# ray-project/anyscale-workshop-nyc-2023

Measured on NVIDIA H100. Metric: generated tokens/sec (and prompts/sec) FLAN-T5-base 512->128, higher is better.
Workload: dtype bf16

## Files before the change

anyscale_workshop_nyc_2023_b200/csrc/attention_encoder.cuh:

```cuda
#pragma once
#include "attention_decode.cuh"
#include "ptx.cuh"

namespace b200 {

constexpr int kEncThreads = 128;
constexpr int kEncQ = 64;
constexpr int kEncKC = 64;
constexpr int kEncPackMaxS = 512;

DEVINL void cp_async_16(uint32_t smem_dst, const void* gsrc, bool valid) {
  const int sz = valid ? 16 : 0;
  asm volatile("cp.async.cg.shared.global [%0], [%1], 16, %2;" ::"r"(smem_dst), "l"(gsrc), "r"(sz) : "memory");
}
DEVINL void cp_async_commit() { asm volatile("cp.async.commit_group;" ::: "memory"); }
template <int N>
DEVINL void cp_async_wait() {
  asm volatile("cp.async.wait_group %0;" ::"n"(N) : "memory");
}
DEVINL void ldmatrix_x4(uint32_t addr, uint32_t& r0, uint32_t& r1, uint32_t& r2, uint32_t& r3) {
  asm volatile("ldmatrix.sync.aligned.m8n8.x4.shared.b16 {%0,%1,%2,%3}, [%4];"
               : "=r"(r0), "=r"(r1), "=r"(r2), "=r"(r3)
               : "r"(addr));
}
// ... 157 lines not shown
          float cm = -INFINITY;
#pragma unroll
          for (int nt = 0; nt < 8; ++nt) cm = fmaxf(cm, fmaxf(sacc[nt][2 * r], sacc[nt][2 * r + 1]));
          cm = fmaxf(cm, __shfl_xor_sync(0xffffffffu, cm, 1));
          cm = fmaxf(cm, __shfl_xor_sync(0xffffffffu, cm, 2));
          const float mn = fmaxf(m_run[r], cm);
          float add = 0.f;
#pragma unroll
          for (int nt = 0; nt < 8; ++nt) add += expf(sacc[nt][2 * r] - mn) + expf(sacc[nt][2 * r + 1] - mn);
          l_run[r] = l_run[r] * expf(m_run[r] - mn) + add;
          m_run[r] = mn;
        }
      } else {
        const uint32_t vbase = sV_u + buf * 8192;
#pragma unroll
        for (int kk = 0; kk < 4; ++kk) {
          uint32_t pa[4];
          pa[0] = pack_act2(expf(sacc[2 * kk][0] - m_run[0]) / l_run[0], expf(sacc[2 * kk][1] - m_run[0]) / l_run[0]);
          pa[1] = pack_act2(expf(sacc[2 * kk][2] - m_run[1]) / l_run[1], expf(sacc[2 * kk][3] - m_run[1]) / l_run[1]);
          pa[2] = pack_act2(expf(sacc[2 * kk + 1][0] - m_run[0]) / l_run[0],
                              expf(sacc[2 * kk + 1][1] - m_run[0]) / l_run[0]);
          pa[3] = pack_act2(expf(sacc[2 * kk + 1][2] - m_run[1]) / l_run[1],
                              expf(sacc[2 * kk + 1][3] - m_run[1]) / l_run[1]);
#pragma unroll
          for (int dp = 0; dp < 4; ++dp) {
            const int mi = lane >> 3;
            const int key = kk * 16 + (mi & 1) * 8 + (lane & 7);
            const int ch = dp * 2 + (mi >> 1);
            uint32_t b0, b1, b2, b3;
            ldmatrix_x4_trans(vbase + tile_off(key, ch), b0, b1, b2, b3);
            mma_act_16816(oacc[2 * dp], pa, b0, b1);
            mma_act_16816(oacc[2 * dp + 1], pa, b2, b3);
          }
        }
      }
      __syncthreads();
    }
  }

#pragma unroll
  for (int r = 0; r < 2; ++r) {
    const int i = i0 + row_l0 + r * 8;
    if (i < rows) {
      act_t* dst = ctx + (row0 + i) * I + h * 64 + tq * 2;
#pragma unroll
      for (int nt = 0; nt < 8; ++nt)
        *reinterpret_cast<uint32_t*>(dst + nt * 8) = pack_act2(oacc[nt][2 * r], oacc[nt][2 * r + 1]);
    }
  }
}

inline size_t encoder_attn_smem_bytes(int S) { return 8192 + 16384 + 16384 + (S + 64) * 4 + S + 16; }

}
```

anyscale_workshop_nyc_2023_b200/csrc/b200t5.cu:

```cuda
#include <cuda.h>
#include <cuda_bf16.h>
#include <cuda_fp16.h>
#include <cuda_runtime.h>
#include <math.h>
#include <stdarg.h>
#include <stdio.h>
#include <string.h>

#include <algorithm>
#include <map>
#include <memory>
#include <string>
#include <vector>

#include "../../include/b200t5.h"
#include "attention_decode.cuh"
#include "attention_cross_stream.cuh"
#include "attention_encoder.cuh"
#include "elementwise.cuh"
#include "gemm.cuh"
#include "gemm_splitk.cuh"
#include "gemm_2cta.cuh"

using namespace b200;
// ... 283 lines not shown
  long long g_eos = -1, g_pad = -1;
  int g_min_new = -1;
  long long* h_ids = nullptr;
  long long* h_mask = nullptr;
  long long* h_out = nullptr;
  int* h_len = nullptr;
  DecodeState* h_state = nullptr;
  ~Plan() {
    if (gexec) cudaGraphExecDestroy(gexec);
    if (graph) cudaGraphDestroy(graph);
    if (gexec8) cudaGraphExecDestroy(gexec8);
    if (graph8) cudaGraphDestroy(graph8);
    if (h_ids) cudaFreeHost(h_ids);
    if (h_mask) cudaFreeHost(h_mask);
    if (h_out) cudaFreeHost(h_out);
    if (h_len) cudaFreeHost(h_len);
    if (h_state) cudaFreeHost(h_state);
    if (h_cu) cudaFreeHost(h_cu);
    if (h_unf) cudaFreeHost(h_unf);
    if (h_admit) cudaFreeHost(h_admit);
  }
};

struct b200t5_ctx {
  Cfg c;
  int device = 0;
  int num_sms = 132;
  bool finalized = false;
  int ffo_k = 0;
  char err[512] = "";
  std::map<std::string, std::unique_ptr<DevBuf>> raw;
  std::map<std::string, std::unique_ptr<DevBuf>> raw_f32;
  std::map<std::string, std::vector<int64_t>> raw_shape;
  DevBuf shared, lm_head, enc_final_ln, dec_final_ln, enc_relbias, dec_relbias, wcrosskv;
  CUtensorMap tm_lm, tm_crosskv, tm2_crosskv;
  std::vector<float> enc_relbias_h, dec_relbias_h;
  std::vector<EncLayerW> enc;
  std::vector<DecLayerW> dec;
  std::unique_ptr<Plan> plan;
  cudaStream_t cap_stream = nullptr, exec_stream = nullptr, enc_stream = nullptr;
  cudaEvent_t enc_done_ev = nullptr, admitted_ev = nullptr;
  bool admit_overlap = true;
  cudaEvent_t ev[4] = {nullptr, nullptr, nullptr, nullptr};
  bool ev_valid = false;
  int pow_mode = 0;
  bool use_pdl = true;
  GeluLut gelu_lut{nullptr, 0, 0};
  struct SkChoice {
    int bn, split;
  };
  bool pack_rows = true;
  bool use_2cta = true;
  bool enc_gemm_ws = true;
  bool self_block = true;
  int xattn_mode = 2;
  int xs_stages = 5;
  bool xs_late_pdl = true;
  bool xs_l2_prefetch = false;
  bool xattn_serialize = false;
  std::vector<cudaEvent_t> xattn_ev;
  bool profile_xattn = false;
  int small_prio = 0;
  bool sk_on = true;
  int sk_stages64 = 0, sk_stages128 = 0;
  SkChoice sk_qkv{64, 2}, sk_proj{64, 4}, sk_wi{128, 2}, sk_ffo{64, 4};
  int chains_override = 0;
  cudaStream_t chain_streams[kMaxChains] = {};
  cudaEvent_t chain_ev[kMaxChains + 1] = {};
  int64_t launches = 0;
  int last_steps = 0;
  double last_decode_bytes = 0, last_enc_flops = 0;
};

static int fail(b200t5_ctx* h, int code, const char* fmt, ...) {
  char buf[512];
  va_list ap;
  va_start(ap, fmt);
  vsnprintf(buf, sizeof(buf), fmt, ap);
  va_end(ap);
  if (h) snprintf(h->err, sizeof(h->err), "%s", buf);
  snprintf(g_err, sizeof(g_err), "%s", buf);
  return code;
}

static int check_device(b200t5_ctx* h, int device) {
  int n = 0;
  cudaError_t e = cudaGetDeviceCount(&n);
  if (e != cudaSuccess || n <= 0)
    return fail(h, B200T5_ENODEV, "no CUDA device available (%s); libb200t5 has no CPU fallback",
                e == cudaSuccess ? "count=0" : cudaGetErrorString(e));
  if (device < 0 || device >= n) return fail(h, B200T5_EINVAL, "device %d out of range (%d devices)", device, n);
  cudaDeviceProp p;
  CU_OK(h, cudaGetDeviceProperties(&p, device));
  if (p.major != 9)
    return fail(h, B200T5_ENODEV, "device %d is sm_%d%d; libb200t5 is built for sm_90a only", device, p.major, p.minor);
  CU_OK(h, cudaSetDevice(device));
  return p.multiProcessorCount;
}

extern "C" int b200t5_relative_bucket(int rel, int bidirectional, int num_buckets, int max_distance) {
  int ret = 0, n;
  if (bidirectional) {
    num_buckets /= 2;
    if (rel > 0) ret += num_buckets;
    n = rel < 0 ? -rel : rel;
  } else {
// ... 82 lines not shown
static cudaError_t run_ffo_sk(b200t5_ctx* h, const b200t5_ctx::SkChoice& ch, const CUtensorMap& tmA, const CUtensorMap& tmB,
                              int M, int N, const EpiResidual::Params& ep, cudaStream_t s, bool pdl) {
  h->launches++;
  constexpr bool tf = B200T5_F16 != 0;
  const int split = splitk_factor(h->ffo_k, ch.split, tf ? kBK / 2 : kBK);
  const int akb = tf ? h->ffo_k / 64 : 0;
  if (ch.bn == 128) return launch_gemm_splitk<128, EpiResidual, tf>(tmA, tmB, M, N, h->ffo_k, split, ep, s, pdl, akb, h->sk_stages128);
  return launch_gemm_splitk<64, EpiResidual, tf>(tmA, tmB, M, N, h->ffo_k, split, ep, s, pdl, akb, h->sk_stages64);
}

static cudaError_t run_rmsnorm(b200t5_ctx* h, const res_t* x, const act_t* w, act_t* y, int M, int d, float eps,
                               cudaStream_t s, bool pdl = false) {
  if (h) h->launches++;
  const int wpb = 8;
  const int grid = (M + wpb - 1) / wpb;
  if (d <= 1024) return launch_kernel(rmsnorm_kernel<4>, dim3(grid), dim3(wpb * 32), 0, s, pdl, x, w, y, M, d, eps);
  if (d <= 4096) return launch_kernel(rmsnorm_kernel<16>, dim3(grid), dim3(wpb * 32), 0, s, pdl, x, w, y, M, d, eps);
  return cudaErrorInvalidValue;
}

static cudaError_t init_kernel_attrs() {
  cudaError_t e;
#define PREP(BN, EPI)                         \
  if ((e = prepare_gemm<BN, EPI>()) != cudaSuccess) return e;
  PREP(256, EpiStore) PREP(256, EpiResidual) PREP(256, EpiGeglu) PREP(256, EpiCrossKV) PREP(64, EpiQkvDecode)
  PREP(32, EpiStore) PREP(32, EpiResidual) PREP(64, EpiGeglu) PREP(128, EpiStoreF32)
  PREP(64, EpiStore) PREP(128, EpiStore)
#undef PREP
  for (const auto& row : kLmHeads)
    for (const LmHead& lh : row)
      if ((e = lh.prepare()) != cudaSuccess) return e;
  if ((e = prepare_gemm_2cta<EpiStore>()) != cudaSuccess) return e;
  if ((e = prepare_gemm_2cta<EpiResidual>()) != cudaSuccess) return e;
  if ((e = prepare_gemm_2cta<EpiGeglu>()) != cudaSuccess) return e;
  if ((e = prepare_gemm_2cta<EpiCrossKV>()) != cudaSuccess) return e;
  if ((e = prepare_gemm_enc_ws<EpiStore>()) != cudaSuccess) return e;
  if ((e = prepare_gemm_enc_ws<EpiResidual>()) != cudaSuccess) return e;
  if ((e = prepare_gemm_enc_ws<EpiGeglu>()) != cudaSuccess) return e;
  if ((e = prepare_gemm_enc_ws<EpiCrossKV>()) != cudaSuccess) return e;
#define PREPSK(BN, EPI) \
  if ((e = prepare_gemm_splitk<BN, EPI>()) != cudaSuccess) return e;
  PREPSK(64, EpiStore) PREPSK(128, EpiStore) PREPSK(64, EpiResidual) PREPSK(128, EpiResidual)
  PREPSK(64, EpiQkvDecode) PREPSK(128, EpiQkvDecode) PREPSK(64, EpiGeglu) PREPSK(128, EpiGeglu)
#undef PREPSK
  if ((e = prepare_gemm_2cta<EpiResidual, B200T5_F16 != 0>()) != cudaSuccess) return e;
  if ((e = prepare_gemm_splitk<64, EpiResidual, B200T5_F16 != 0>()) != cudaSuccess) return e;
  if ((e = prepare_gemm_splitk<128, EpiResidual, B200T5_F16 != 0>()) != cudaSuccess) return e;
  if ((e = cudaFuncSetAttribute(self_attn_decode_warp_kernel, cudaFuncAttributeMaxDynamicSharedMemorySize,
                                kSelfWarpsPerCta * 4096 * 4)) != cudaSuccess)
    return e;
  if ((e = cudaFuncSetAttribute(attn_cross_stream_kernel, cudaFuncAttributeMaxDynamicSharedMemorySize,
                                static_cast<int>(XsSmem::bytes(kXsMaxStages, 4096)))) != cudaSuccess)
    return e;
  return cudaFuncSetAttribute(encoder_attn_kernel, cudaFuncAttributeMaxDynamicSharedMemorySize, 96 * 1024);
}

struct GeluLutOwner {
  DevBuf table;
  GeluLut lut{nullptr, 0, 0};
  int pow_mode = -1;
};
static GeluLutOwner g_gelu;

[[maybe_unused]] static int ensure_gelu_lut(b200t5_ctx* h, int pow_mode, GeluLut* out) {
  if (g_gelu.lut.table && g_gelu.pow_mode == pow_mode) {
    *out = g_gelu.lut;
    return B200T5_OK;
  }
  DevBuf full;
  CU_OK(h, full.alloc(65536 * 2));
  build_gelu_table_kernel<<<256, 256>>>(full.as<uint16_t>(), pow_mode);
  CU_OK(h, cudaGetLastError());
  std::vector<uint16_t> t(65536);
  CU_OK(h, cudaMemcpy(t.data(), full.p, 65536 * 2, cudaMemcpyDeviceToHost));
  auto half_bits = [](uint16_t xb) {
    uint32_t u = static_cast<uint32_t>(xb) << 16;
    float f;
    memcpy(&f, &u, 4);
    f *= 0.5f;
    memcpy(&u, &f, 4);
    u += 0x7FFFu + ((u >> 16) & 1u);
    return static_cast<uint16_t>(u >> 16);
  };
  int lo = 0;
  while (lo < 0x7F80 && t[lo] == half_bits(static_cast<uint16_t>(lo)) && t[0x8000 | lo] == half_bits(static_cast<uint16_t>(0x8000 | lo))) ++lo;
  int hi = 0x7F80;
  while (hi > lo && t[hi - 1] == static_cast<uint16_t>(hi - 1) && t[0x8000 | (hi - 1)] == 0x8000) --hi;
  const int n = hi - lo;
  if (n < 0 || 2 * n * 2 > kEpiSmemBytes) return fail(h, B200T5_ECUDA, "gelu table window [%#x,%#x) does not fit the epilogue scratch", lo, hi);
  std::vector<uint16_t> compact(((static_cast<size_t>(2) * (n > 0 ? n : 1) + 7) / 8) * 8 + 8, 0);
  for (int i = 0; i < n; ++i) {
    compact[i] = t[lo + i];
    compact[n + i] = t[0x8000 | (lo + i)];
  }
  CU_OK(h, g_gelu.table.alloc(compact.size() * 2));
  CU_OK(h, cudaMemcpy(g_gelu.table.p, compact.data(), compact.size() * 2, cudaMemcpyHostToDevice));
  g_gelu.lut = GeluLut{g_gelu.table.as<uint16_t>(), lo, hi};
  g_gelu.pow_mode = pow_mode;
  *out = g_gelu.lut;
  return B200T5_OK;
}

extern "C" const char* b200t5_version(void) {
  return B200T5_F16 ? "b200t5 0.1 fp16 (sm_90a, wgmma/TMA)" : "b200t5 0.1 (sm_90a, wgmma/TMA)";
}
extern "C" const char* b200t5_last_global_error(void) { return g_err; }
extern "C" const char* b200t5_last_error(b200t5_handle h) { return h ? h->err : g_err; }

extern "C" int b200t5_create(const b200t5_config* cfg, int device, b200t5_handle* out) {
  if (!cfg || !out) return fail(nullptr, B200T5_EINVAL, "null argument");
  *out = nullptr;
  if (cfg->d_kv != 64) return fail(nullptr, B200T5_EINVAL, "d_kv=%d unsupported (kernels are specialised for 64)", cfg->d_kv);
  if (!cfg->is_gated_gelu) return fail(nullptr, B200T5_EINVAL, "only feed_forward_proj='gated-gelu' (T5 v1.1 / FLAN-T5) is supported");
  if (cfg->scale_decoder_outputs) return fail(nullptr, B200T5_EINVAL, "scale_decoder_outputs (tied-embedding T5 v1.0) is not supported");
  if (cfg->d_model % 8 || cfg->d_ff % 32 || cfg->d_model > 4096 || cfg->vocab_size < 2 || cfg->num_heads < 1 ||
      cfg->num_layers < 1 || cfg->num_decoder_layers < 1)
    return fail(nullptr, B200T5_EINVAL, "unsupported shape: d_model=%d d_ff=%d vocab=%d", cfg->d_model, cfg->d_ff, cfg->vocab_size);
  int sms = check_device(nullptr, device);
  if (sms < 0) return sms;
  b200t5_ctx* h = new (std::nothrow) b200t5_ctx();
  if (!h) return fail(nullptr, B200T5_ENOMEM, "out of host memory");
  h->c = Cfg{cfg->vocab_size, cfg->d_model, cfg->d_ff, cfg->num_heads, cfg->num_heads * 64, cfg->num_layers,
             cfg->num_decoder_layers, cfg->relative_attention_num_buckets, cfg->relative_attention_max_distance,
             cfg->layer_norm_epsilon, cfg->pad_token_id, cfg->eos_token_id, cfg->decoder_start_token_id};
  h->device = device;
  h->num_sms = sms;
  h->enc.resize(h->c.Le);
  h->dec.resize(h->c.Ld);
  const char* pm = getenv("B200T5_POW_MODE");
  h->pow_mode = pm ? atoi(pm) : 0;
  const char* pdl_env = getenv("B200T5_PDL");
  h->use_pdl = pdl_env ? atoi(pdl_env) != 0 : true;
  if (const char* pr_env = getenv("B200T5_PRIO")) h->small_prio = atoi(pr_env);
  if (const char* pk_env = getenv("B200T5_PACK")) h->pack_rows = atoi(pk_env) != 0;
  if (const char* tc_env = getenv("B200T5_2CTA")) h->use_2cta = atoi(tc_env) != 0;
  if (const char* eg_env = getenv("B200T5_ENC_GEMM")) h->enc_gemm_ws = atoi(eg_env) != 0;
  if (const char* sf_env = getenv("B200T5_SELF")) h->self_block = strcmp(sf_env, "warp") != 0;
  if (const char* xa_env = getenv("B200T5_XATTN")) h->xattn_mode = strcmp(xa_env, "ldg") == 0 ? 0 : strcmp(xa_env, "stream") == 0 ? 1 : 2;
  if (const char* xs_env = getenv("B200T5_XS_STAGES")) {
    const int v = atoi(xs_env);
    if (v >= 2 && v <= kXsMaxStages) h->xs_stages = v;
  }
  if (const char* lp_env = getenv("B200T5_XS_LATE_PDL")) h->xs_late_pdl = atoi(lp_env) != 0;
  if (const char* se_env = getenv("B200T5_XS_SERIALIZE")) h->xattn_serialize = atoi(se_env) != 0;
  if (const char* pf_env = getenv("B200T5_XS_L2PF")) h->xs_l2_prefetch = atoi(pf_env) != 0;
  if (const char* sk_env = getenv("B200T5_SK")) {
    int v[8];
    const int n = sscanf(sk_env, "%d,%d,%d,%d,%d,%d,%d,%d", &v[0], &v[1], &v[2], &v[3], &v[4], &v[5], &v[6], &v[7]);
    if (n == 1 && v[0] == 0) h->sk_on = false;
    if (n == 8) {
      b200t5_ctx::SkChoice* dst[4] = {&h->sk_qkv, &h->sk_proj, &h->sk_wi, &h->sk_ffo};
      for (int i = 0; i < 4; ++i) {
        dst[i]->bn = v[2 * i] == 128 ? 128 : 64;
        dst[i]->split = v[2 * i + 1] >= 8 ? 8 : (v[2 * i + 1] >= 4 ? 4 : (v[2 * i + 1] >= 2 ? 2 : 1));
      }
    }
  }
  if (const char* st_env = getenv("B200T5_SK_STAGES")) {
    int a = 0, b = 0;
    if (sscanf(st_env, "%d,%d", &a, &b) == 2) {
      h->sk_stages64 = a;
      h->sk_stages128 = b;
    }
  }
  const char* ch_env = getenv("B200T5_CHAINS");
  h->chains_override = ch_env ? atoi(ch_env) : 0;
#if B200T5_F16
  h->use_2cta = h->pack_rows = true;
  if (!h->sk_on) {
    delete h;
    return fail(nullptr, B200T5_EINVAL, "B200T5_SK=0 is not available in the fp16 build");
  }
#endif
  if (const char* ao_env = getenv("B200T5_ADMIT_OVERLAP")) h->admit_overlap = atoi(ao_env) != 0;
  int prio_lo = 0, prio_hi = 0;
  cudaDeviceGetStreamPriorityRange(&prio_lo, &prio_hi);
  if (cudaStreamCreateWithFlags(&h->cap_stream, cudaStreamNonBlocking) != cudaSuccess ||
      cudaStreamCreateWithFlags(&h->exec_stream, cudaStreamNonBlocking) != cudaSuccess ||
      cudaStreamCreateWithPriority(&h->enc_stream, cudaStreamNonBlocking, prio_lo) != cudaSuccess ||
      cudaEventCreateWithFlags(&h->enc_done_ev, cudaEventDisableTiming) != cudaSuccess ||
      cudaEventCreateWithFlags(&h->admitted_ev, cudaEventDisableTiming) != cudaSuccess) {
    delete h;
    return fail(nullptr, B200T5_ECUDA, "cudaStreamCreate failed");
  }
  {
    cudaError_t ke = init_kernel_attrs();
    if (ke != cudaSuccess) {
      delete h;
      return fail(nullptr, B200T5_ECUDA, "kernel attribute setup failed: %s", cudaGetErrorString(ke));
// ... 392 lines not shown
}

static GemmOp mk(const CUtensorMap& a, const CUtensorMap& b, int M, int N, int K, GemmKind k, int m_fastest) {
  GemmOp g;
  g.tmA = a;
  g.tmB = b;
  g.M = M;
  g.N = N;
  g.K = K;
  g.kind = k;
  g.m_fastest = m_fastest;
  return g;
}

static int run_encoder(b200t5_ctx* h, const long long* ids, const long long* mask, cudaStream_t s, const int* row_on = nullptr) {
  const Cfg& c = h->c;
  Plan& p = *h->plan;
  const int B = p.B, S = p.S, d = c.d, I = c.I, F = c.F, H = c.H;
  int M = B * S;
  prep_mask_kernel<<<B, 128, 0, s>>>(mask, p.key_ok.as<unsigned char>(), p.extent.as<int>(), B, S, row_on);
  h->launches++;
  p.packed = h->pack_rows && S <= kEncPackMaxS;
  if (row_on && !p.packed)
    return fail(h, B200T5_EINVAL, "slot-pool admission needs the packed encoder path (S <= %d, B200T5_PACK at its default)", kEncPackMaxS);
  const int* cu = nullptr;
  p.rows_valid = M;
  if (p.packed) {
    pack_offsets_kernel<<<1, 256, 0, s>>>(p.extent.as<int>(), p.cu.as<int>(), B);
    CU_OK(h, cudaMemcpyAsync(p.h_cu, p.cu.as<int>() + B, 4, cudaMemcpyDeviceToHost, s));
    CU_OK(h, cudaStreamSynchronize(s));
    M = *p.h_cu;
    p.rows_valid = M;
    cu = p.cu.as<int>();
    embed_rows_packed_kernel<<<dim3((S + 7) / 8, B), 256, 0, s>>>(ids, h->shared.as<act_t>(), p.x.as<res_t>(), cu, p.row_b.as<int>(),
                                                               p.row_s.as<int>(), S, d, c.V);
    h->launches += 2;
  } else {
    embed_rows_kernel<<<(M + 7) / 8, 256, 0, s>>>(ids, h->shared.as<act_t>(), p.x.as<res_t>(), M, d, c.V);
    h->launches++;
  }
  p.packed_rows = M;
  CU_OK(h, cudaGetLastError());
  const size_t attn_smem = encoder_attn_smem_bytes(S);
  if (attn_smem > 96 * 1024) return fail(h, B200T5_EINVAL, "encoder length S=%d too long for the attention kernel", S);
  const int wi_tiles = (F + 127) / 128;
  for (int l = 0; l < c.Le; ++l) {
    EncLayerW& w = h->enc[l];
    CU_OK(h, run_rmsnorm(h, p.x.as<res_t>(), w.ln0.as<act_t>(), p.xn.as<act_t>(), M, d, c.eps, s));
    {
      EpiStore::Params ep{p.qkv.as<act_t>(), 3 * I};
      if (h->use_2cta) CU_OK(h, run_gemm_2cta<EpiStore>(h, p.tm_xn, w.tm2_qkv, M, 3 * I, d, ep, s));
      else CU_OK(h, run_gemm(h, mk(p.tm_xn, w.tm_qkv, M, 3 * I, d, G_STORE256, 0), &ep, s));
    }
    encoder_attn_kernel<<<dim3((S + kEncQ - 1) / kEncQ, B * H), kEncThreads, attn_smem, s>>>(
        p.qkv.as<act_t>(), p.ctx.as<act_t>(), p.enc_bias.as<float>(), p.key_ok.as<unsigned char>(), p.extent.as<int>(), cu, S, H);
    h->launches++;
    CU_OK(h, cudaGetLastError());
    {
      EpiResidual::Params ep{p.x.as<res_t>(), p.x.as<res_t>(), d};
      ep.round_out = l == 0;
      if (h->use_2cta) CU_OK(h, run_gemm_2cta<EpiResidual>(h, p.tm_ctx, w.tm2_o, M, d, I, ep, s));
      else CU_OK(h, run_gemm(h, mk(p.tm_ctx, w.tm_o, M, d, I, G_RES256, 0), &ep, s));
    }
    CU_OK(h, run_rmsnorm(h, p.x.as<res_t>(), w.ln1.as<act_t>(), p.xn.as<act_t>(), M, d, c.eps, s));
    {
      EpiGeglu::Params ep{p.hff.as<ffh_t>(), F, h->gelu_lut};
      if (h->use_2cta) CU_OK(h, run_gemm_2cta<EpiGeglu>(h, p.tm_xn, w.tm2_wi, M, wi_tiles * 256, d, ep, s));
      else CU_OK(h, run_gemm(h, mk(p.tm_xn, w.tm_wi, M, wi_tiles * 256, d, G_GEGLU256, 0), &ep, s));
    }
    {
      EpiResidual::Params ep{p.x.as<res_t>(), p.x.as<res_t>(), d};
      ep.round_acc = B200T5_F16 ? 0 : 1;
      ep.round_out = B200T5_F16 ? 0 : 1;
      if (h->use_2cta) CU_OK(h, run_ffo_2cta(h, p.tm_hff, w.tm2_ffo, M, d, ep, s));
      else CU_OK(h, run_gemm(h, mk(p.tm_hff, w.tm_ffo, M, d, F, G_RES256, 0), &ep, s));
    }
  }
  CU_OK(h, run_rmsnorm(h, p.x.as<res_t>(), h->enc_final_ln.as<act_t>(), p.xn.as<act_t>(), M, d, c.eps, s));
  return B200T5_OK;
}

static int run_cross_kv(b200t5_ctx* h, cudaStream_t s) {
  const Cfg& c = h->c;
  Plan& p = *h->plan;
  EpiCrossKV::Params ep{p.cross_kv.as<act_t>(), p.B, c.H, p.S};
  if (p.packed) {
    ep.row_b = p.row_b.as<int>();
    ep.row_s = p.row_s.as<int>();
  }
  const int M = p.packed ? p.packed_rows : p.B * p.S;
  if (h->use_2cta) CU_OK(h, run_gemm_2cta<EpiCrossKV>(h, p.tm_xn, h->tm2_crosskv, M, c.Ld * 2 * c.I, c.d, ep, s));
  else CU_OK(h, run_gemm(h, mk(p.tm_xn, h->tm_crosskv, M, c.Ld * 2 * c.I, c.d, G_CROSSKV256, 0), &ep, s));
  return B200T5_OK;
}

struct ChainView {
  int b0, nb;
  res_t* dx;
  ffh_t* dh;
  act_t *dxn, *dq, *dctx;
  const Plan::Chain* ch;
};
static ChainView chain_view(b200t5_ctx* h, const Plan::Chain& ch) {
  Plan& p = *h->plan;
  const Cfg& c = h->c;
  ChainView v;
  v.b0 = ch.b0;
  v.nb = ch.nb;
// ... 799 lines not shown
                                               p.dctx.as<act_t>() + static_cast<size_t>(b0) * c.I, p.extent.as<int>() + b0,
                                               p.key_ok.as<unsigned char>() + static_cast<size_t>(b0) * p.S, -1);
        if (e != cudaSuccess) le = e;
        ++launches;
      }
    }
  };
  sweep();
  CU_OK(h, le);
  cudaEvent_t e0 = nullptr, e1 = nullptr;
  struct EvGuard {
    cudaEvent_t &a, &b;
    ~EvGuard() {
      if (a) cudaEventDestroy(a);
      if (b) cudaEventDestroy(b);
    }
  } guard{e0, e1};
  CU_OK(h, cudaEventCreate(&e0));
  CU_OK(h, cudaEventCreate(&e1));
  CU_OK(h, cudaEventRecord(e0, s));
  for (int r = 0; r < reps; ++r) sweep();
  CU_OK(h, cudaEventRecord(e1, s));
  CU_OK(h, cudaEventSynchronize(e1));
  CU_OK(h, le);
  float ms = 0.f;
  CU_OK(h, cudaEventElapsedTime(&ms, e0, e1));
  CU_OK(h, cudaGetLastError());
  *avg_ms_per_launch = ms / (static_cast<float>(reps) * launches);
  std::vector<int> ext(p.B);
  CU_OK(h, cudaMemcpy(ext.data(), p.extent.p, p.B * 4, cudaMemcpyDeviceToHost));
  double sum_s = 0;
  for (int v : ext) sum_s += v;
  *bytes_per_launch = 2.0 * 2.0 * c.I * sum_s / (static_cast<double>(launches) / c.Ld);
  return B200T5_OK;
}

extern "C" int b200t5_set_option(b200t5_handle h, const char* name, int value) {
  if (!h || !name) return fail(h, B200T5_EINVAL, "null argument");
  const std::string n(name);
  if (n == "chains") h->chains_override = value < 0 ? 0 : value;
  else if (n == "xattn") h->xattn_mode = value < 0 || value > 2 ? 2 : value;
  else if (n == "xattn_stages") {
    if (value < 2 || value > kXsMaxStages) return fail(h, B200T5_EINVAL, "xattn_stages must be in [2, %d]", kXsMaxStages);
    h->xs_stages = value;
  } else if (n == "xattn_late_pdl") h->xs_late_pdl = value != 0;
  else if (n == "xattn_serialize") h->xattn_serialize = value != 0;
  else if (n == "xattn_l2pf") h->xs_l2_prefetch = value != 0;
  else if (n == "pdl") h->use_pdl = value != 0;
  else if (n == "admit_overlap") h->admit_overlap = value != 0;
  else if (n == "sk_stages64") h->sk_stages64 = value;
  else if (n == "sk_stages128") h->sk_stages128 = value;
  else if (n == "profile_xattn") h->profile_xattn = value != 0;
  else if (n == "enc_gemm") h->enc_gemm_ws = value != 0;
  else return fail(h, B200T5_EINVAL, "unknown option '%s'", name);
  CU_OK(h, cudaSetDevice(h->device));
  CU_OK(h, cudaDeviceSynchronize());
  h->plan.reset();
  return B200T5_OK;
}

extern "C" int b200t5_get_xattn_profile(b200t5_handle h, double* avg_us_per_launch, int64_t* launches, double* bytes_per_launch,
                                        double* busy_us_per_layer, double* bytes_per_layer) {
  if (!h || !avg_us_per_launch || !launches || !bytes_per_launch || !busy_us_per_layer || !bytes_per_layer)
    return fail(h, B200T5_EINVAL, "null argument");
  if (!h->plan || !h->profile_xattn) return fail(h, B200T5_ESTATE, "profiling is off (b200t5_set_option(h, \"profile_xattn\", 1), then generate)");
  CU_OK(h, cudaSetDevice(h->device));
  CU_OK(h, cudaDeviceSynchronize());
  Plan& p = *h->plan;
  const int n = h->c.Ld * p.n_chains;
  std::vector<unsigned long long> acc(static_cast<size_t>(n + h->c.Ld) * 2);
  CU_OK(h, cudaMemcpy(acc.data(), p.xs_acc.p, acc.size() * 8, cudaMemcpyDeviceToHost));
  unsigned long long ns = 0, cnt = 0, busy = 0, layers = 0;
  for (int i = 0; i < n; ++i) {
    ns += acc[2 * i];
    cnt += acc[2 * i + 1];
  }
  for (int l = 0; l < h->c.Ld; ++l) {
    busy += acc[2 * (n + l)];
    layers += acc[2 * (n + l) + 1];
  }
  *avg_us_per_launch = cnt ? static_cast<double>(ns) / static_cast<double>(cnt) / 1e3 : 0.0;
  *busy_us_per_layer = layers ? static_cast<double>(busy) / static_cast<double>(layers) / 1e3 : 0.0;
  *launches = static_cast<int64_t>(cnt);
  std::vector<int> ext(p.B);
  CU_OK(h, cudaMemcpy(ext.data(), p.extent.p, p.B * 4, cudaMemcpyDeviceToHost));
  double sum_s = 0;
  for (int v : ext) sum_s += v;
  *bytes_per_layer = 2.0 * 2.0 * h->c.I * sum_s;
  *bytes_per_launch = *bytes_per_layer / p.n_chains;
  return B200T5_OK;
}

extern "C" int b200t5_encode(b200t5_handle h, const int64_t* input_ids, const int64_t* attention_mask, int B, int S,
                             void* enc_out_bf16, void* stream) {
  TRY(validate(h, B, S, nullptr));
  if (!input_ids || !enc_out_bf16) return fail(h, B200T5_EINVAL, "null argument");
  CU_OK(h, cudaSetDevice(h->device));
  cudaStream_t s = static_cast<cudaStream_t>(stream);
  const int T = h->plan && h->plan->B == B && h->plan->S == S ? h->plan->Tmax : 1;
  TRY(ensure_plan(h, B, S, T));
  TRY(run_encoder(h, reinterpret_cast<const long long*>(input_ids), reinterpret_cast<const long long*>(attention_mask), s));
  if (h->plan->packed) {
    unpack_rows_kernel<<<dim3((S + 7) / 8, B), 256, 0, s>>>(h->plan->xn.as<act_t>(), h->plan->cu.as<int>(), static_cast<act_t*>(enc_out_bf16), S, h->c.d);
    CU_OK(h, cudaGetLastError());
  } else {
    CU_OK(h, cudaMemcpyAsync(enc_out_bf16, h->plan->xn.p, static_cast<size_t>(B) * S * h->c.d * 2, cudaMemcpyDeviceToDevice, s));
// ... 326 lines not shown
  cudaError_t e = run_rmsnorm(nullptr, static_cast<const act_t*>(x), static_cast<const act_t*>(w), static_cast<act_t*>(y), M, d, eps, static_cast<cudaStream_t>(stream));
  if (e != cudaSuccess) return fail(nullptr, B200T5_ECUDA, "rmsnorm: %s", cudaGetErrorString(e));
  return B200T5_OK;
#endif
}

extern "C" int b200t5_test_attn_decode(int device, int self, const void* q, const void* K, const void* V, void* ctx,
                                       int B, int H, int Tk, const int32_t* extent, const uint8_t* key_ok, int step,
                                       const float* dist_bias, void* stream) {
#if B200T5_F16
  return fail(nullptr, B200T5_EINVAL, "the single-kernel test hooks exist in the bf16 build only (libb200t5.so)");
#else
  const int sms = hook_device(device);
  if (sms < 0) return sms;
  cudaStream_t s = static_cast<cudaStream_t>(stream);
  if (self == 1) {
    DevBuf st;
    if (st.alloc(sizeof(DecodeState)) != cudaSuccess) return fail(nullptr, B200T5_ECUDA, "alloc");
    set_state_kernel<<<1, 1, 0, s>>>(st.as<DecodeState>(), step);
    self_attn_decode_warp_kernel<<<(B * H + kSelfWarpsPerCta - 1) / kSelfWarpsPerCta, kSelfWarpsPerCta * 32,
                                   kSelfWarpsPerCta * Tk * sizeof(float), s>>>(
        static_cast<const act_t*>(q), static_cast<const act_t*>(K), static_cast<const act_t*>(V), static_cast<act_t*>(ctx),
        B * H, H, Tk, &st.as<DecodeState>()->step, dist_bias);
    cudaStreamSynchronize(s);
  } else if (self == 2) {
    const int stages = step > 0 ? step : 5;
    if (stages < 2 || stages > kXsMaxStages || Tk > 4096) return fail(nullptr, B200T5_EINVAL, "attn_decode(stream): 2 <= stages <= %d, Tk <= 4096", kXsMaxStages);
    const int items = B * H;
    CUtensorMap tk, tv;
    if (!make_tmap(&tk, K, static_cast<uint64_t>(items) * Tk, 64, kXsChunkKeys) || !make_tmap(&tv, V, static_cast<uint64_t>(items) * Tk, 64, kXsChunkKeys))
      return fail(nullptr, B200T5_ECUDA, "%s", g_err);
    attn_cross_stream_kernel<<<xs_grid(items, sms), kXsThreads, XsSmem::bytes(stages, Tk), s>>>(
        tk, tv, 0, 0, static_cast<const act_t*>(K), static_cast<const act_t*>(V), static_cast<const act_t*>(q), static_cast<act_t*>(ctx), items, H,
        Tk, extent, key_ok, stages, 1, 1, XsStamps{nullptr, 0});
  } else {
    attn_decode_kernel<false><<<B * H, kAttnDecThreads, Tk * sizeof(float), s>>>(
        static_cast<const act_t*>(q), static_cast<const act_t*>(K), static_cast<const act_t*>(V), static_cast<act_t*>(ctx), H,
        Tk, extent, key_ok, nullptr, nullptr, XsStamps{nullptr, 0});
  }
  cudaError_t e = cudaGetLastError();
  if (e != cudaSuccess) return fail(nullptr, B200T5_ECUDA, "attn_decode: %s", cudaGetErrorString(e));
  return B200T5_OK;
#endif
}

extern "C" int b200t5_test_encoder_attn(int device, const void* qkv, void* ctx, const float* rel_bias,
                                        const uint8_t* key_ok, const int32_t* extent, int B, int S, int H, int impl,
                                        void* stream) {
#if B200T5_F16
  return fail(nullptr, B200T5_EINVAL, "the single-kernel test hooks exist in the bf16 build only (libb200t5.so)");
#else
  const int sms = hook_device(device);
  if (sms < 0) return sms;
  DevBuf cu;
  if (impl == 1) {
    std::vector<int> hcu(B);
    for (int b = 0; b < B; ++b) hcu[b] = b * S;
    if (cu.alloc(B * sizeof(int)) != cudaSuccess || cudaMemcpy(cu.p, hcu.data(), B * sizeof(int), cudaMemcpyHostToDevice) != cudaSuccess)
      return fail(nullptr, B200T5_ECUDA, "encoder_attn: offsets");
  }
  const size_t smem = encoder_attn_smem_bytes(S);
  cudaError_t e = smem <= 96 * 1024 ? cudaSuccess : cudaErrorInvalidValue;
  if (e == cudaSuccess) {
    encoder_attn_kernel<<<dim3((S + kEncQ - 1) / kEncQ, B * H), kEncThreads, smem, static_cast<cudaStream_t>(stream)>>>(
        static_cast<const act_t*>(qkv), static_cast<act_t*>(ctx), rel_bias, key_ok, extent, impl == 1 ? cu.as<int>() : nullptr, S, H);
    e = cudaGetLastError();
  }
  if (e != cudaSuccess) return fail(nullptr, B200T5_ECUDA, "encoder_attn: %s", cudaGetErrorString(e));
  return B200T5_OK;
#endif
}

extern "C" int b200t5_test_geglu(int device, const void* gate, const void* up, void* out, int64_t n, int pow_mode, void* stream) {
#if B200T5_F16
  return fail(nullptr, B200T5_EINVAL, "the single-kernel test hooks exist in the bf16 build only (libb200t5.so)");
#else
  const int sms = hook_device(device);
  if (sms < 0) return sms;
  GeluLut lut;
  int lrc = ensure_gelu_lut(nullptr, 0, &lut);
  if (lrc != B200T5_OK) return lrc;
  geglu_elementwise_kernel<<<static_cast<unsigned>((n + 255) / 256), 256, 0, static_cast<cudaStream_t>(stream)>>>(
      static_cast<const act_t*>(gate), static_cast<const act_t*>(up), static_cast<act_t*>(out), n, pow_mode, lut);
  cudaError_t e = cudaGetLastError();
  if (e != cudaSuccess) return fail(nullptr, B200T5_ECUDA, "geglu: %s", cudaGetErrorString(e));
  return B200T5_OK;
#endif
}
```

Baseline: 82640.

## Add one-pass encoder attention kernel that caches scores in shared memory

Adds a one-pass encoder attention kernel. The QK^T scores for all key chunks are computed once, stored as packed bf16 in shared memory, and later read back to form normalized probabilities for the PV product. The old kernel recomputed QK^T and reloaded K in a second pass. The new kernel also uses a precomputed per-chunk 'fully valid' flag to skip the masking branches, and it reuses the Q and score slots to hold V tiles. In exchange it uses up to about 227KB of shared memory per block, which limits occupancy to one block per SM, and the V-slot scheduling is more intricate.

Result: faster. 83470 (median of 6 runs) (+1.0%).

```diff
diff --git a/anyscale_workshop_nyc_2023_b200/csrc/attention_encoder.cuh b/anyscale_workshop_nyc_2023_b200/csrc/attention_encoder.cuh
--- a/anyscale_workshop_nyc_2023_b200/csrc/attention_encoder.cuh
+++ b/anyscale_workshop_nyc_2023_b200/csrc/attention_encoder.cuh
@@ -233,4 +233,235 @@
 
 inline size_t encoder_attn_smem_bytes(int S) { return 8192 + 16384 + 16384 + (S + 64) * 4 + S + 16; }
 
-}
+constexpr int kEnc1pMaxSmem = 227 * 1024;
+constexpr size_t enc1p_slots_bytes(int S) { return static_cast<size_t>((S + kEncKC - 1) / kEncKC + 1) * 8192; }
+constexpr size_t encoder_attn_1p_smem_bytes(int S) {
+  return enc1p_slots_bytes(S) + static_cast<size_t>(S + 64) * 4 + S + (S + kEncKC - 1) / kEncKC;
+}
+constexpr int enc1p_max_s() {
+  int s = kEncKC;
+  while (encoder_attn_1p_smem_bytes(s + kEncKC) <= kEnc1pMaxSmem) s += kEncKC;
+  return s;
+}
+constexpr int kEnc1pMaxS = enc1p_max_s();
+
+__global__ void __launch_bounds__(kEncThreads)
+encoder_attn_1p_kernel(const act_t* __restrict__ qkv, act_t* __restrict__ ctx, const float* __restrict__ rel_bias,
+                       const unsigned char* __restrict__ key_ok, const int* __restrict__ extent, const int* __restrict__ cu,
+                       int S, int H) {
+  extern __shared__ __align__(128) uint8_t enc_smem[];
+  const int I = H * 64;
+  const int ld = 3 * I;
+  const int bh = blockIdx.y;
+  const int b = bh / H, h = bh - b * H;
+  const int i0 = blockIdx.x * kEncQ;
+  const int warp = threadIdx.x >> 5, lane = threadIdx.x & 31;
+  const int g = lane >> 2, tq = lane & 3;
+
+  float* sBias = reinterpret_cast<float*>(enc_smem + enc1p_slots_bytes(S));
+  unsigned char* sOk = reinterpret_cast<unsigned char*>(sBias + S + 64);
+  unsigned char* sFull = sOk + S;
+  const uint32_t slot0 = smem_u32(enc_smem);
+
+  const int ext = extent[b];
+  const int rows = cu ? ext : S;
+  if (i0 >= rows) return;
+  const size_t row0 = cu ? static_cast<size_t>(cu[b]) : static_cast<size_t>(b) * S;
+  const int nchunks = (ext + kEncKC - 1) / kEncKC;
+  const act_t* qg = qkv + row0 * ld + h * 64;
+  const act_t* kg = qg + I;
+  const act_t* vg = qg + 2 * I;
+
+  auto k_slot = [&](int c) { return slot0 + (c + 1) * 8192; };
+  auto v_slot = [&](int c) { return (c & 1) ? slot0 : slot0 + nchunks * 8192; };
+  auto load_k = [&](int c) { load_tile_async(k_slot(c), kg, ld, c * kEncKC, min(kEncKC, ext - c * kEncKC)); };
+  auto load_v = [&](int c) { load_tile_async(v_slot(c), vg, ld, c * kEncKC, min(kEncKC, ext - c * kEncKC)); };
+
+  {
+    const int lo = S - 64 - i0;
+    for (int x = threadIdx.x; x < S + 63; x += kEncThreads) {
+      const int idx = lo + x;
+      sBias[x] = (idx >= 0 && idx < 2 * S - 1) ? rel_bias[static_cast<size_t>(h) * (2 * S - 1) + idx] : 0.f;
+    }
+    for (int x = threadIdx.x; x < S; x += kEncThreads) sOk[x] = key_ok[static_cast<size_t>(b) * S + x];
+    if (warp == 0) {
+      for (int c = 0; c < nchunks; ++c) {
+        const int j = c * kEncKC + lane * 2;
+        const unsigned char* ok = key_ok + static_cast<size_t>(b) * S + j;
+        const bool full = __all_sync(0xffffffffu, j + 1 < ext && ok[0] && ok[1]);
+        if (lane == 0) sFull[c] = full;
+      }
+    }
+  }
+  load_tile_async(slot0, qg, ld, i0, min(kEncQ, rows - i0));
+  load_k(0);
+  cp_async_commit();
+
+  float m_run[2] = {-INFINITY, -INFINITY};
+  float l_run[2] = {0.f, 0.f};
+  const int row_l0 = warp * 16 + g;
+  const uint32_t my_scores = slot0 + warp * 2048 + lane * 16;
+
+  {
+    uint32_t qa[4][4];
+    for (int c = 0; c < nchunks; ++c) {
+      cp_async_wait<0>();
+      __syncthreads();
+      if (c + 1 < nchunks) {
+        load_k(c + 1);
+        cp_async_commit();
+      }
+      if (c == 0) {
+#pragma unroll
+        for (int kk = 0; kk < 4; ++kk) {
+          const int r = warp * 16 + (lane & 15);
+          const int ch = kk * 2 + (lane >> 4);
+          ldmatrix_x4(slot0 + tile_off(r, ch), qa[kk][0], qa[kk][1], qa[kk][2], qa[kk][3]);
+        }
+      }
+
+      float sacc[8][4];
+#pragma unroll
+      for (int nt = 0; nt < 8; ++nt)
+#pragma unroll
+        for (int e = 0; e < 4; ++e) sacc[nt][e] = 0.f;
+      const uint32_t kbase = k_slot(c);
+#pragma unroll
+      for (int kk = 0; kk < 4; ++kk) {
+#pragma unroll
+        for (int np = 0; np < 4; ++np) {
+          const int mi = lane >> 3;
+          const int key = np * 16 + (mi >> 1) * 8 + (lane & 7);
+          const int ch = kk * 2 + (mi & 1);
+          uint32_t b0, b1, b2, b3;
+          ldmatrix_x4(kbase + tile_off(key, ch), b0, b1, b2, b3);
+          mma_act_16816(sacc[2 * np], qa[kk], b0, b1);
+          mma_act_16816(sacc[2 * np + 1], qa[kk], b2, b3);
+        }
+      }
+
+      const int jc = c * kEncKC;
+      const float* bias = sBias + jc + tq * 2 - row_l0 + 63;
+      if (sFull[c]) {
+#pragma unroll
+        for (int nt = 0; nt < 8; ++nt)
+#pragma unroll
+          for (int e = 0; e < 4; ++e) sacc[nt][e] = act_round(act_round(sacc[nt][e]) + bias[nt * 8 + (e & 1) - (e >> 1) * 8]);
+      } else {
+#pragma unroll
+        for (int nt = 0; nt < 8; ++nt) {
+#pragma unroll
+          for (int e = 0; e < 4; ++e) {
+            const int j = jc + nt * 8 + tq * 2 + (e & 1);
+            float s = act_round(sacc[nt][e]);
+            if (j < ext) {
+              s = act_round(s + bias[nt * 8 + (e & 1) - (e >> 1) * 8]);
+              if (!sOk[j]) s = kActMin;
+            } else {
+              s = -INFINITY;
+            }
+            sacc[nt][e] = s;
+          }
+        }
+      }
+
+#pragma unroll
+      for (int r = 0; r < 2; ++r) {
+        float cm = -INFINITY;
+#pragma unroll
+        for (int nt = 0; nt < 8; ++nt) cm = fmaxf(cm, fmaxf(sacc[nt][2 * r], sacc[nt][2 * r + 1]));
+        cm = fmaxf(cm, __shfl_xor_sync(0xffffffffu, cm, 1));
+        cm = fmaxf(cm, __shfl_xor_sync(0xffffffffu, cm, 2));
+        const float mn = fmaxf(m_run[r], cm);
+        float add = 0.f;
+#pragma unroll
+        for (int nt = 0; nt < 8; ++nt) add += expf(sacc[nt][2 * r] - mn) + expf(sacc[nt][2 * r + 1] - mn);
+        l_run[r] = l_run[r] * expf(m_run[r] - mn) + add;
+        m_run[r] = mn;
+      }
+
+      if (c == 0) __syncwarp();
+#pragma unroll
+      for (int kk = 0; kk < 4; ++kk) {
+        const uint32_t a = my_scores + c * 8192 + kk * 512;
+        asm volatile("st.shared.v4.b32 [%0], {%1, %2, %3, %4};" ::"r"(a),
+                     "r"(pack_act2(sacc[2 * kk][0], sacc[2 * kk][1])), "r"(pack_act2(sacc[2 * kk][2], sacc[2 * kk][3])),
+                     "r"(pack_act2(sacc[2 * kk + 1][0], sacc[2 * kk + 1][1])), "r"(pack_act2(sacc[2 * kk + 1][2], sacc[2 * kk + 1][3]))
+                     : "memory");
+      }
+    }
+  }
+  __syncthreads();
+  if (nchunks > 0) {
+    load_v(0);
+    cp_async_commit();
+  }
+#pragma unroll
+  for (int r = 0; r < 2; ++r) {
+    l_run[r] += __shfl_xor_sync(0xffffffffu, l_run[r], 1);
+    l_run[r] += __shfl_xor_sync(0xffffffffu, l_run[r], 2);
+  }
+
+  float oacc[8][4];
+#pragma unroll
+  for (int nt = 0; nt < 8; ++nt)
+#pragma unroll
+    for (int e = 0; e < 4; ++e) oacc[nt][e] = 0.f;
+  for (int c = 0; c < nchunks; ++c) {
+    if (c == 1) {
+      __syncthreads();
+      load_v(1);
+      cp_async_commit();
+      if (nchunks > 2) {
+        load_v(2);
+        cp_async_commit();
+        cp_async_wait<1>();
+      } else {
+        cp_async_wait<0>();
+      }
+    } else {
+      cp_async_wait<0>();
+    }
+    __syncthreads();
+    if (c >= 2 && c + 1 < nchunks) {
+      load_v(c + 1);
+      cp_async_commit();
+    }
+    const uint32_t vbase = v_slot(c);
+#pragma unroll
+    for (int kk = 0; kk < 4; ++kk) {
+      uint32_t w0, w1, w2, w3;
+      asm volatile("ld.shared.v4.b32 {%0, %1, %2, %3}, [%4];"
+                   : "=r"(w0), "=r"(w1), "=r"(w2), "=r"(w3)
+                   : "r"(my_scores + c * 8192 + kk * 512));
+      uint32_t pa[4];
+      pa[0] = pack_act2(expf(act_lo(w0) - m_run[0]) / l_run[0], expf(act_hi(w0) - m_run[0]) / l_run[0]);
+      pa[1] = pack_act2(expf(act_lo(w1) - m_run[1]) / l_run[1], expf(act_hi(w1) - m_run[1]) / l_run[1]);
+      pa[2] = pack_act2(expf(act_lo(w2) - m_run[0]) / l_run[0], expf(act_hi(w2) - m_run[0]) / l_run[0]);
+      pa[3] = pack_act2(expf(act_lo(w3) - m_run[1]) / l_run[1], expf(act_hi(w3) - m_run[1]) / l_run[1]);
+#pragma unroll
+      for (int dp = 0; dp < 4; ++dp) {
+        const int mi = lane >> 3;
+        const int key = kk * 16 + (mi & 1) * 8 + (lane & 7);
+        const int ch = dp * 2 + (mi >> 1);
+        uint32_t b0, b1, b2, b3;
+        ldmatrix_x4_trans(vbase + tile_off(key, ch), b0, b1, b2, b3);
+        mma_act_16816(oacc[2 * dp], pa, b0, b1);
+        mma_act_16816(oacc[2 * dp + 1], pa, b2, b3);
+      }
+    }
+  }
+
+#pragma unroll
+  for (int r = 0; r < 2; ++r) {
+    const int i = i0 + row_l0 + r * 8;
+    if (i < rows) {
+      act_t* dst = ctx + (row0 + i) * I + h * 64 + tq * 2;
+#pragma unroll
+      for (int nt = 0; nt < 8; ++nt)
+        *reinterpret_cast<uint32_t*>(dst + nt * 8) = pack_act2(oacc[nt][2 * r], oacc[nt][2 * r + 1]);
+    }
+  }
+}
+
+}
diff --git a/anyscale_workshop_nyc_2023_b200/csrc/b200t5.cu b/anyscale_workshop_nyc_2023_b200/csrc/b200t5.cu
--- a/anyscale_workshop_nyc_2023_b200/csrc/b200t5.cu
+++ b/anyscale_workshop_nyc_2023_b200/csrc/b200t5.cu
@@ -359,6 +359,7 @@
   bool pack_rows = true;
   bool use_2cta = true;
   bool enc_gemm_ws = true;
+  bool enc_attn_1p = true;
   bool self_block = true;
   int xattn_mode = 2;
   int xs_stages = 5;
@@ -547,7 +548,21 @@
   if ((e = cudaFuncSetAttribute(attn_cross_stream_kernel, cudaFuncAttributeMaxDynamicSharedMemorySize,
                                 static_cast<int>(XsSmem::bytes(kXsMaxStages, 4096)))) != cudaSuccess)
     return e;
+  if ((e = cudaFuncSetAttribute(encoder_attn_1p_kernel, cudaFuncAttributeMaxDynamicSharedMemorySize, kEnc1pMaxSmem)) != cudaSuccess)
+    return e;
+  if ((e = cudaFuncSetAttribute(encoder_attn_1p_kernel, cudaFuncAttributePreferredSharedMemoryCarveout,
+                                cudaSharedmemCarveoutMaxShared)) != cudaSuccess)
+    return e;
   return cudaFuncSetAttribute(encoder_attn_kernel, cudaFuncAttributeMaxDynamicSharedMemorySize, 96 * 1024);
+}
+
+static void launch_encoder_attn(bool one_pass, const act_t* qkv, act_t* ctx, const float* rel_bias, const unsigned char* key_ok,
+                                const int* extent, const int* cu, int B, int S, int H, cudaStream_t s) {
+  const dim3 grid((S + kEncQ - 1) / kEncQ, B * H);
+  if (one_pass && S <= kEnc1pMaxS)
+    encoder_attn_1p_kernel<<<grid, kEncThreads, encoder_attn_1p_smem_bytes(S), s>>>(qkv, ctx, rel_bias, key_ok, extent, cu, S, H);
+  else
+    encoder_attn_kernel<<<grid, kEncThreads, encoder_attn_smem_bytes(S), s>>>(qkv, ctx, rel_bias, key_ok, extent, cu, S, H);
 }
 
 struct GeluLutOwner {
@@ -630,6 +645,7 @@
   if (const char* pk_env = getenv("B200T5_PACK")) h->pack_rows = atoi(pk_env) != 0;
   if (const char* tc_env = getenv("B200T5_2CTA")) h->use_2cta = atoi(tc_env) != 0;
   if (const char* eg_env = getenv("B200T5_ENC_GEMM")) h->enc_gemm_ws = atoi(eg_env) != 0;
+  if (const char* ea_env = getenv("B200T5_ENC_ATTN")) h->enc_attn_1p = atoi(ea_env) != 0;
   if (const char* sf_env = getenv("B200T5_SELF")) h->self_block = strcmp(sf_env, "warp") != 0;
   if (const char* xa_env = getenv("B200T5_XATTN")) h->xattn_mode = strcmp(xa_env, "ldg") == 0 ? 0 : strcmp(xa_env, "stream") == 0 ? 1 : 2;
   if (const char* xs_env = getenv("B200T5_XS_STAGES")) {
@@ -1128,8 +1144,8 @@
       if (h->use_2cta) CU_OK(h, run_gemm_2cta<EpiStore>(h, p.tm_xn, w.tm2_qkv, M, 3 * I, d, ep, s));
       else CU_OK(h, run_gemm(h, mk(p.tm_xn, w.tm_qkv, M, 3 * I, d, G_STORE256, 0), &ep, s));
     }
-    encoder_attn_kernel<<<dim3((S + kEncQ - 1) / kEncQ, B * H), kEncThreads, attn_smem, s>>>(
-        p.qkv.as<act_t>(), p.ctx.as<act_t>(), p.enc_bias.as<float>(), p.key_ok.as<unsigned char>(), p.extent.as<int>(), cu, S, H);
+    launch_encoder_attn(h->enc_attn_1p, p.qkv.as<act_t>(), p.ctx.as<act_t>(), p.enc_bias.as<float>(), p.key_ok.as<unsigned char>(),
+                        p.extent.as<int>(), cu, B, S, H, s);
     h->launches++;
     CU_OK(h, cudaGetLastError());
     {
@@ -2035,6 +2051,7 @@
   else if (n == "sk_stages128") h->sk_stages128 = value;
   else if (n == "profile_xattn") h->profile_xattn = value != 0;
   else if (n == "enc_gemm") h->enc_gemm_ws = value != 0;
+  else if (n == "enc_attn") h->enc_attn_1p = value != 0;
   else return fail(h, B200T5_EINVAL, "unknown option '%s'", name);
   CU_OK(h, cudaSetDevice(h->device));
   CU_OK(h, cudaDeviceSynchronize());
@@ -2467,8 +2484,9 @@
 #else
   const int sms = hook_device(device);
   if (sms < 0) return sms;
+  const bool packed = impl & 1, one_pass = !(impl & 2);
   DevBuf cu;
-  if (impl == 1) {
+  if (packed) {
     std::vector<int> hcu(B);
     for (int b = 0; b < B; ++b) hcu[b] = b * S;
     if (cu.alloc(B * sizeof(int)) != cudaSuccess || cudaMemcpy(cu.p, hcu.data(), B * sizeof(int), cudaMemcpyHostToDevice) != cudaSuccess)
@@ -2477,8 +2495,8 @@
   const size_t smem = encoder_attn_smem_bytes(S);
   cudaError_t e = smem <= 96 * 1024 ? cudaSuccess : cudaErrorInvalidValue;
   if (e == cudaSuccess) {
-    encoder_attn_kernel<<<dim3((S + kEncQ - 1) / kEncQ, B * H), kEncThreads, smem, static_cast<cudaStream_t>(stream)>>>(
-        static_cast<const act_t*>(qkv), static_cast<act_t*>(ctx), rel_bias, key_ok, extent, impl == 1 ? cu.as<int>() : nullptr, S, H);
+    launch_encoder_attn(one_pass, static_cast<const act_t*>(qkv), static_cast<act_t*>(ctx), rel_bias, key_ok, extent,
+                        packed ? cu.as<int>() : nullptr, B, S, H, static_cast<cudaStream_t>(stream));
     e = cudaGetLastError();
   }
   if (e != cudaSuccess) return fail(nullptr, B200T5_ECUDA, "encoder_attn: %s", cudaGetErrorString(e));
```
